# Vandermode/ELD

Measured on NVIDIA H100. Metric: raw frames/sec (noise+U-Net), higher is better.
Workload: dtype bf16

## Files before the change

eld_b200/csrc/conv3x3_thin.cuh:

```cuda
#pragma once
#include "conv_gemm.cuh"

namespace eld {

__host__ __device__ constexpr int thin_stg_bytes(int nt) { return 128 * nt * 2; }
constexpr int kThinMaxSlots = 4;
constexpr int kThinSmemBytes = 227 * 1024;

__device__ __forceinline__ uint32_t thin_stg_off(int m, int q) { return (uint32_t)(m * 64 + ((q ^ ((m >> 1) & 3)) << 4)); }

template <int NT, int KC>
__global__ void __launch_bounds__(kConvThreads, 1)
conv3x3_thin_kernel(const __grid_constant__ CUtensorMap tmA, const __grid_constant__ CUtensorMap tmOut,
                    const __grid_constant__ CUtensorMap tmOut2, const ConvGemmParams p)
{
    extern __shared__ uint8_t smem_raw[];
    const uint32_t raw = ptx::smem_u32(smem_raw);
    uint8_t* smem = smem_raw + (((raw + 1023u) & ~1023u) - raw);

    constexpr int row_bytes = KC * 2;
    constexpr int tap_bytes = NT * row_bytes;
    constexpr int slot_bytes = halo_slot_bytes(KC);
    constexpr int NC = NT / 32;
    uint8_t* b_s = smem;
    uint8_t* slots = smem + 9 * tap_bytes;
    uint64_t* full = reinterpret_cast<uint64_t*>(smem + p.bar_smem_off);
    uint64_t* empty = full + p.stages;
    uint64_t* b_full = empty + p.stages;
    float* s_bias = reinterpret_cast<float*>(smem + p.bias_smem_off);

    const int total_tiles = p.n_img * p.tiles_y * p.tiles_x;
    const int tiles_xy = p.tiles_x * p.tiles_y;

    if (threadIdx.x == 0) {
        ptx::prefetch_tmap(&tmA);
        ptx::prefetch_tmap(&tmOut);
        for (int s = 0; s < p.stages; ++s) { ptx::mbar_init(&full[s], 1); ptx::mbar_init(&empty[s], 4); }
        ptx::mbar_init(b_full, 1);
        ptx::fence_barrier_init();
    }
    if (p.bias)
        for (int i = threadIdx.x; i < p.n_total; i += kConvThreads) s_bias[i] = __ldg(p.bias + i);
    __syncthreads();
    ptx::grid_dep_wait();
    ptx::grid_dep_launch();

    if (threadIdx.x < 128) {
        if (threadIdx.x == 0) {
            ptx::mbar_arrive_expect_tx(b_full, (uint32_t)(9 * tap_bytes));
            for (int tap = 0; tap < 9; ++tap)
                ptx::bulk_load(b_s + tap * tap_bytes, p.b_ptr + (size_t)tap * p.b_rows * row_bytes, (uint32_t)tap_bytes, b_full);
            int s = 0;
            uint32_t ph = 0;
            for (int tile = blockIdx.x; tile < total_tiles; tile += gridDim.x) {
                const int img = tile / tiles_xy;
                const int rem = tile - img * tiles_xy;
                const int ty = rem / p.tiles_x, tx = rem - ty * p.tiles_x;
                const int x0 = tx * kConvTileW, y0 = ty * 8;
                ptx::mbar_wait(&empty[s], ph ^ 1u);
                uint8_t* sa = slots + (size_t)s * slot_bytes;
                ptx::mbar_arrive_expect_tx(&full[s], (uint32_t)slot_bytes);
                halo_load<KC>(sa, &tmA, &full[s], p.a_c0, x0, y0, img);
                if (++s == p.stages) { s = 0; ph ^= 1u; }
            }
        }
        return;
    }

    const int cg = __shfl_sync(0xffffffffu, (int)(threadIdx.x >> 7) - 1, 0);
    const int t = threadIdx.x & 127;
    const int lane = threadIdx.x & 31;
    const uint32_t layout = ptx::gmma_layout(row_bytes);
    const uint64_t desc0 = ptx::make_gmma_desc(0, 16, 8u * row_bytes, layout);
    const uint32_t b_base = ptx::smem_u32(b_s), slot_base = ptx::smem_u32(slots);
    uint8_t* stg = smem + p.stg_smem_off + cg * thin_stg_bytes(NT);
    const uint32_t stg_base = ptx::smem_u32(stg);
    const int wq = t >> 5, lr = lane >> 2, q = lane & 3;
    const size_t n_pix = (size_t)p.n_img * p.H * p.W;
    float bias[NT / 8][2];
#pragma unroll
    for (int j = 0; j < NT / 8; ++j) { bias[j][0] = p.bias ? s_bias[8 * j + 2 * q] : 0.f; bias[j][1] = p.bias ? s_bias[8 * j + 2 * q + 1] : 0.f; }
    ptx::mbar_wait(b_full, 0);
    for (int jt = cg;; jt += 2) {
        const int tile = blockIdx.x + jt * gridDim.x;
        if (tile >= total_tiles) break;
        const int s = jt % p.stages;
        const int img = tile / tiles_xy;
        const int rem = tile - img * tiles_xy;
        const int ty = rem / p.tiles_x, tx = rem - ty * p.tiles_x;
        const int x0 = tx * kConvTileW, y0 = ty * 8;
        long long pix[4];
#pragma unroll
        for (int u = 0; u < 4; ++u) {
            const int x = x0 + lr + 8 * (u & 1), y = y0 + 4 * (u >> 1) + wq;
            pix[u] = (x < p.W && y < p.H) ? ((long long)(img * p.H + y) * p.W + x) : -1;
        }
        ptx::mbar_wait(&full[s], (uint32_t)(jt / p.stages) & 1u);
        float acc[2][NT / 2];
        const uint32_t sa = slot_base + (uint32_t)(s * slot_bytes);
        ptx::wgmma_fence();
#pragma unroll
        for (int tap = 0; tap < 9; ++tap) {
            const uint32_t a_addr = sa + halo_tap_off(KC, tap);
            const uint64_t bd = ptx::desc_at(desc0, b_base + (uint32_t)(tap * tap_bytes));
#pragma unroll
            for (int k = 0; k < KC / 16; ++k) {
#pragma unroll
                for (int h = 0; h < 2; ++h) {
                    const uint64_t ad = ptx::desc_at(desc0, a_addr + (uint32_t)(h * 64 * row_bytes));
                    ptx::wgmma_bf16<NT, 0, 0>(acc[h], ad + 2u * k, bd + 2u * k, (tap | k) != 0 ? 1u : 0u);
                }
            }
        }
        ptx::wgmma_commit();
        uint32_t mneg[4][NC], mtie[4][NC];
        if (p.act == ACT_MASK && p.aux_slope) {
#pragma unroll
            for (int u = 0; u < 4; ++u)
#pragma unroll
                for (int c = 0; c < NC; ++c) {
                    const uint32_t* sw = p.aux_slope + (size_t)pix[u] * NC + c;
                    mneg[u][c] = pix[u] >= 0 ? __ldg(sw) : 0u;
                    mtie[u][c] = pix[u] >= 0 ? __ldg(sw + n_pix * NC) : 0u;
                }
        }
        ptx::wgmma_wait<0>();
        ptx::reg_fence(acc[0]);
        ptx::reg_fence(acc[1]);
        if (lane == 0) ptx::mbar_arrive(&empty[s]);

        if (p.act == ACT_MASK && !p.aux_slope) {
#pragma unroll
            for (int u = 0; u < 4; ++u)
#pragma unroll
                for (int c = 0; c < NC; ++c) {
                    mneg[u][c] = 0u; mtie[u][c] = 0u;
#pragma unroll
                    for (int jj = 0; jj < 4; ++jj) {
                        if (pix[u] < 0) continue;
                        const int k = 4 * jj + q;
                        const uint32_t w = __ldg(reinterpret_cast<const uint32_t*>(
                            p.aux + (size_t)pix[u] * p.aux_pitch + (p.aux_c0 + 32 * c + 2 * k)));
                        uint32_t n, tc;
                        ptx::slope_classes(w, n, tc);
                        mneg[u][c] |= (n >> (15 - k)) & (0x00010001u << k);
                        mtie[u][c] |= (tc >> (15 - k)) & (0x00010001u << k);
                    }
                }
        }

        uint32_t wv[2][NT / 8][2];
#pragma unroll
        for (int h = 0; h < 2; ++h)
#pragma unroll
            for (int j = 0; j < NT / 8; ++j)
#pragma unroll
                for (int i = 0; i < 2; ++i) {
                    float v[2] = { acc[h][4 * j + 2 * i], acc[h][4 * j + 2 * i + 1] };
#pragma unroll
                    for (int c = 0; c < 2; ++c) {
                        if (p.bias) v[c] += bias[j][c];
                        if (p.act == ACT_LRELU) {
                            v[c] = fmaxf(v[c], 0.2f * v[c]);
                        } else if (p.act == ACT_MASK) {
                            const int u = 2 * h + i, b = 4 * (j & 3) + q + 16 * c;
                            v[c] *= lrelu_slope(mneg[u][j >> 2], mtie[u][j >> 2], b, kMaskNeg);
                        }
                    }
                    const __nv_bfloat162 b2 = __floats2bfloat162_rn(v[0], v[1]);
                    wv[h][j][i] = *reinterpret_cast<const uint32_t*>(&b2);
                }
        if (p.slope_out) {
            uint32_t sn[4][NC], st[4][NC];
#pragma unroll
            for (int u = 0; u < 4; ++u)
#pragma unroll
                for (int c = 0; c < NC; ++c) {
                    sn[u][c] = 0u; st[u][c] = 0u;
#pragma unroll
                    for (int jj = 0; jj < 4; ++jj) {
                        const int k = 4 * jj + q;
                        uint32_t n, tc;
                        ptx::slope_classes(wv[u >> 1][4 * c + jj][u & 1], n, tc);
                        sn[u][c] |= (n >> (15 - k)) & (0x00010001u << k);
                        st[u][c] |= (tc >> (15 - k)) & (0x00010001u << k);
                    }
#pragma unroll
                    for (int o = 1; o <= 2; o <<= 1) {
                        sn[u][c] |= __shfl_xor_sync(0xffffffffu, sn[u][c], o);
                        st[u][c] |= __shfl_xor_sync(0xffffffffu, st[u][c], o);
                    }
                }
#pragma unroll
            for (int u = 0; u < 4; ++u)
                if (u == q && pix[u] >= 0) {
                    uint32_t* sw = p.slope_out + (size_t)pix[u] * NC;
#pragma unroll
                    for (int c = 0; c < NC; ++c) { sw[c] = sn[u][c]; sw[n_pix * NC + c] = st[u][c]; }
                }
        }

        if (t == 0) ptx::bulk_wait_read<0>();
        ptx::bar_sync(1 + cg, 128);
#pragma unroll
        for (int h = 0; h < 2; ++h)
#pragma unroll
            for (int c = 0; c < NC; ++c)
#pragma unroll
                for (int jp = 0; jp < 2; ++jp) {
                    const int g = lane >> 3;
                    const int m = 64 * h + 16 * wq + 8 * (g & 1) + (lane & 7);
                    const int j0 = 4 * c + 2 * jp;
                    ptx::stmatrix_x4(stg_base + (uint32_t)(c * 128 * 64) + thin_stg_off(m, 2 * jp + (g >> 1)),
                                     wv[h][j0][0], wv[h][j0][1], wv[h][j0 + 1][0], wv[h][j0 + 1][1]);
                }
        ptx::fence_proxy_async();
        ptx::bar_sync(1 + cg, 128);
        if (t == 0) {
#pragma unroll
            for (int c = 0; c < NC; ++c) {
                const bool second = p.out_split && 32 * c >= p.out_split;
                ptx::tma_store_5d(second ? &tmOut2 : &tmOut, stg + c * 128 * 64,
                                  second ? 32 * c - p.out_split : p.out_c0 + 32 * c, x0, y0, img, 0);
            }
            ptx::bulk_commit();
        }
        if (p.pool_out) {
#pragma unroll
            for (int it = t; it < 128 * NC; it += 128) {
                const int qq = it & 3, px = (it >> 2) & 7, py = (it >> 5) & 3, c = it >> 7;
                const uint8_t* blk = stg + c * 128 * 64;
                uint32_t w[4][4];
#pragma unroll
                for (int d = 0; d < 4; ++d) {
                    const uint4 v = *reinterpret_cast<const uint4*>(blk + thin_stg_off(16 * (2 * py + (d >> 1)) + 2 * px + (d & 1), qq));
                    w[d][0] = v.x; w[d][1] = v.y; w[d][2] = v.z; w[d][3] = v.w;
                }
                uint32_t pw[4];
#pragma unroll
                for (int jj = 0; jj < 4; ++jj) pw[jj] = bf2_max(bf2_max(w[0][jj], w[1][jj]), bf2_max(w[2][jj], w[3][jj]));
                const int x = x0 + 2 * px, y = y0 + 2 * py;
                const bool in_img = x < p.W && y < p.H;
                const size_t ppix = (size_t)(img * (p.H >> 1) + (y >> 1)) * (p.W >> 1) + (x >> 1);
                if (in_img)
                    *reinterpret_cast<uint4*>(p.pool_out + ppix * p.pool_pitch + 32 * c + 8 * qq) = make_uint4(pw[0], pw[1], pw[2], pw[3]);
                if (p.pool_code) {
                    uint32_t code[12];
#pragma unroll
                    for (int d = 0; d < 4; ++d) {
                        code[d] = 0u; code[4 + d] = 0u; code[8 + d] = 0u;
#pragma unroll
                        for (int jj = 0; jj < 4; ++jj) {
                            const int k = 4 * qq + jj;
                            const uint32_t ne = __hne2_mask(*reinterpret_cast<const __nv_bfloat162*>(&w[d][jj]),
                                                            *reinterpret_cast<const __nv_bfloat162*>(&pw[jj]));
                            uint32_t n, tc;
                            ptx::slope_classes(w[d][jj], n, tc);
                            code[d] |= (ne >> (15 - k)) & (0x00010001u << k);
                            code[4 + d] |= (n >> (15 - k)) & (0x00010001u << k);
                            code[8 + d] |= (tc >> (15 - k)) & (0x00010001u << k);
                        }
                    }
#pragma unroll
                    for (int e = 0; e < 12; ++e) {
                        code[e] |= __shfl_xor_sync(0xffffffffu, code[e], 1);
                        code[e] |= __shfl_xor_sync(0xffffffffu, code[e], 2);
                    }
                    const size_t rec = ppix * (size_t)(p.pool_pitch >> 5) + (size_t)c;
                    const size_t recs = (size_t)p.n_img * (p.H >> 1) * (p.W >> 1) * (size_t)(p.pool_pitch >> 5);
                    uint32_t* dst = qq == 2 ? p.pool_code + recs * 8 + rec * 4 : p.pool_code + rec * 8 + 4 * qq;
#pragma unroll
                    for (int g = 0; g < 3; ++g)
                        if (in_img && qq == g)
                            *reinterpret_cast<uint4*>(dst) = make_uint4(code[4 * g], code[4 * g + 1], code[4 * g + 2], code[4 * g + 3]);
                }
            }
        }
    }
    if (t == 0) ptx::bulk_wait<0>();
}

}
```

eld_b200/csrc/unet_prims.cu:

```cuda
#include "common.cuh"
#include <algorithm>
#include <cstdlib>
#include <cstdio>
#include "conv_gemm.cuh"
#include "conv3x3_thin.cuh"
#include "conv3x3_wide.cuh"
#include "wgrad_gemm.cuh"
#include "wgrad_thin.cuh"
#include "first_conv.cuh"
#include "unet_prims.h"

namespace eld {

using ConvKernel = void (*)(CUtensorMap, ConvGemmParams);
using WgradKernel = void (*)(CUtensorMap, CUtensorMap, WgradParams);
using WgradThinKernel = void (*)(CUtensorMap, CUtensorMap, WgradThinParams);
using FirstConvKernel = void (*)(CUtensorMap, CUtensorMap, FirstConvParams);
static const ConvKernel kConvGemm[3] = { conv_gemm_kernel<32>, conv_gemm_kernel<64>, conv_gemm_kernel<128> };
using ConvThinKernel = void (*)(CUtensorMap, CUtensorMap, CUtensorMap, ConvGemmParams);
static const ConvThinKernel kConvThin[2][2] = { { conv3x3_thin_kernel<32, 32>, conv3x3_thin_kernel<32, 64> },
                                                { conv3x3_thin_kernel<64, 32>, conv3x3_thin_kernel<64, 64> } };
static const ConvKernel kConvWide[3][2] = { { conv3x3_wide_kernel<32, 32>, conv3x3_wide_kernel<32, 64> },
                                            { conv3x3_wide_kernel<64, 32>, conv3x3_wide_kernel<64, 64> },
                                            { conv3x3_wide_kernel<128, 32>, conv3x3_wide_kernel<128, 64> } };
static const WgradKernel kWgradGemm[3] = { wgrad_gemm_kernel<32>, wgrad_gemm_kernel<64>, wgrad_gemm_kernel<128> };
static const WgradThinKernel kWgradThin[2][2] = { { conv3x3_wgrad_thin_kernel<32, 32>, conv3x3_wgrad_thin_kernel<32, 64> },
                                                  { conv3x3_wgrad_thin_kernel<64, 32>, conv3x3_wgrad_thin_kernel<64, 64> } };
static const FirstConvKernel kFirstConv[2] = { first_conv_kernel<false>, first_conv_kernel<true> };

static int encode(eld_ctx* ctx, CUtensorMap* map, const void* ptr, int rank, const cuuint64_t* dims,
                  const cuuint64_t* strides_bytes, const cuuint32_t* box, int inner_bytes,
                  CUtensorMapDataType dtype = CU_TENSOR_MAP_DATA_TYPE_BFLOAT16)
{
    cuuint32_t estr[5] = { 1, 1, 1, 1, 1 };
    CUtensorMapSwizzle sw = inner_bytes == 128 ? CU_TENSOR_MAP_SWIZZLE_128B
                          : inner_bytes == 64  ? CU_TENSOR_MAP_SWIZZLE_64B
                          : inner_bytes == 32  ? CU_TENSOR_MAP_SWIZZLE_32B : CU_TENSOR_MAP_SWIZZLE_NONE;
    CUresult r = ctx->encode_tiled(map, dtype, (cuuint32_t)rank, const_cast<void*>(ptr),
                                   dims, strides_bytes, box, estr, CU_TENSOR_MAP_INTERLEAVE_NONE, sw,
                                   CU_TENSOR_MAP_L2_PROMOTION_L2_256B, CU_TENSOR_MAP_FLOAT_OOB_FILL_NONE);
    if (r != CUDA_SUCCESS) {
        set_error("cuTensorMapEncodeTiled failed (%d): rank %d dims %llu,%llu,%llu box %u,%u,%u inner %d B",
                  (int)r, rank, (unsigned long long)dims[0], (unsigned long long)dims[1],
                  (unsigned long long)(rank > 2 ? dims[2] : 0), box[0], box[1], rank > 2 ? box[2] : 0, inner_bytes);
        return ELD_E_CUDA;
    }
    return ELD_OK;
}

static int encode_nhwc(eld_ctx* ctx, CUtensorMap* map, const void* t, int pitch, int n, int H, int W,
                       int box_c, int box_w, int box_h)
{
    const cuuint64_t eb = 2;
    cuuint64_t dims[5] = { (cuuint64_t)pitch, (cuuint64_t)W, (cuuint64_t)H, (cuuint64_t)n, 1 };
    cuuint64_t str[4] = { pitch * eb, (cuuint64_t)W * pitch * eb, (cuuint64_t)H * W * pitch * eb,
                          (cuuint64_t)n * H * W * pitch * eb };
    cuuint32_t box[5] = { (cuuint32_t)box_c, (cuuint32_t)box_w, (cuuint32_t)box_h, 1, 1 };
    return encode(ctx, map, t, 5, dims, str, box, box_c * 2);
}

static int encode_subpixel(eld_ctx* ctx, CUtensorMap* map, const void* t, int pitch, int n, int H, int W,
                           int box_c, int box_rows)
{
    const cuuint64_t eb = 2;
    cuuint64_t dims[5] = { (cuuint64_t)pitch, 2, (cuuint64_t)W, 2, (cuuint64_t)n * H };
    cuuint64_t str[4] = { pitch * eb, 2 * pitch * eb, (cuuint64_t)2 * W * pitch * eb, (cuuint64_t)4 * W * pitch * eb };
    cuuint32_t box[5] = { (cuuint32_t)box_c, 1, 16, 1, (cuuint32_t)box_rows };
    return encode(ctx, map, t, 5, dims, str, box, box_c * 2);
}

template <typename Kernel, typename... Args>
static int launch(eld_ctx* ctx, Kernel kernel, int grid, int block, size_t smem, cudaStream_t st, Args... args)
{
    ELD_CHECK_CUDA(launch_pdl(kernel, grid, block, smem, st, args...));
    ELD_CHECK_CUDA(cudaGetLastError());
    count_launch(ctx);
    return ELD_OK;
}

static int conv_gemm_params(const GemmOp& op, ConvGemmParams& p)
{
    const int n_total = op.kind == GEMM_DECONV ? 4 * op.cout : op.cout;
    const bool store = op.kind != GEMM_DECONV;
    ELD_REQUIRE(op.cin % 32 == 0, "conv tile: cin=%d must be a multiple of 32", op.cin);
    ELD_REQUIRE(n_total % 32 == 0, "conv tile: GEMM N=%d must be a multiple of 32", n_total);
    ELD_REQUIRE(op.a_pitch % 8 == 0, "conv tile: the input pitch must be a multiple of 8 channels");
    ELD_REQUIRE(op.out_pitch % 16 == 0 && op.out_c0 % 16 == 0 && (reinterpret_cast<uintptr_t>(op.out) & 31) == 0,
                "conv tile: output pitch / first channel must be multiples of 16 channels and the tensor 32-byte aligned");
    ELD_REQUIRE(op.aux == nullptr || (op.aux_pitch % 16 == 0 && op.aux_c0 % 16 == 0 && (reinterpret_cast<uintptr_t>(op.aux) & 31) == 0),
                "conv tile: mask-source pitch / first channel must be multiples of 16 channels and the tensor 32-byte aligned");
    ELD_REQUIRE(op.pool_out == nullptr || (op.pool_pitch % 16 == 0 && (reinterpret_cast<uintptr_t>(op.pool_out) & 31) == 0),
                "conv tile: pooled-output pitch must be a multiple of 16 channels and the tensor 32-byte aligned");
    p.n_img = op.n_img; p.H = op.H; p.W = op.W;
    p.tiles_x = (op.W + 15) / 16; p.tiles_y = (op.H + 7) / 8;
    p.taps = op.kind == GEMM_CONV3X3 ? 9 : op.kind == GEMM_DECONV ? 1 : 4;
    p.a_mode = op.kind == GEMM_DECONV_DGRAD ? A_GATHER : A_CONV;
    p.cin = op.cin; p.a_c0 = op.a_c0;
    p.kc = (op.cin % 64 == 0) ? 64 : 32;
    p.n_total = n_total;
    p.epi_mode = store ? EPI_STORE : EPI_SHUFFLE; p.act = op.act;
    p.out = static_cast<__nv_bfloat16*>(op.out); p.out_pitch = op.out_pitch; p.out_c0 = op.out_c0;
    p.bias = op.bias;
    p.aux = static_cast<const __nv_bfloat16*>(op.aux); p.aux_pitch = op.aux_pitch; p.aux_c0 = op.aux_c0;
    ELD_REQUIRE(op.aux_slope == nullptr || (op.act == ACT_MASK && store), "conv tile: slope words are a mask source of a plain store epilogue");
    ELD_REQUIRE(op.slope_out == nullptr || (op.act == ACT_LRELU && store && op.out_split == 0),
                "conv tile: slope words are written behind LeakyReLU by a plain store epilogue");
    p.aux_slope = static_cast<const uint32_t*>(op.aux_slope); p.slope_out = static_cast<uint32_t*>(op.slope_out);
    p.cout = op.cout;
    ELD_REQUIRE(op.pool_out == nullptr || (store && op.H % 2 == 0 && op.W % 2 == 0),
                "conv tile: the fused max pool needs a plain store epilogue and even H, W");
    p.pool_out = static_cast<__nv_bfloat16*>(op.pool_out); p.pool_pitch = op.pool_pitch;
    ELD_REQUIRE(op.pool_code == nullptr || (op.pool_out && op.pool_pitch % 32 == 0 && (reinterpret_cast<uintptr_t>(op.pool_code) & 31) == 0),
                "conv tile: the pool code needs the fused pool, a multiple of 32 channels and a 32-byte aligned buffer");
    p.pool_code = static_cast<uint32_t*>(op.pool_code);
    ELD_REQUIRE(op.out_split == 0 || (store && op.out2 && op.out_split % 32 == 0 && op.out2_pitch % 16 == 0 &&
                                     (reinterpret_cast<uintptr_t>(op.out2) & 31) == 0),
                "conv tile: split store needs a plain store epilogue, a second tensor and a split at a multiple of 32 columns");
    p.out2 = static_cast<__nv_bfloat16*>(op.out2); p.out2_pitch = op.out2_pitch; p.out_split = op.out_split;
    ELD_REQUIRE(op.b_block_rows == 0 || (op.b_block_rows % 32 == 0 && op.b_block_rows <= 256 &&
                                         (n_total <= op.b_block_rows || op.b_block_rows == 256) && op.aux_slope == nullptr),
                "conv tile: a row prefix of the packed operand needs whole 32-row groups of its blocks and no slope-word mask");
    ELD_REQUIRE(op.b_block_rows != 0 || n_total <= 256 || n_total % 256 == 0,
                "conv tile: GEMM N=%d above 256 must be a multiple of 256", n_total);
    p.b_rows = op.b_block_rows ? op.b_block_rows : (n_total <= 256 ? n_total : 256);
    p.n_tile = (n_total % 128 == 0) ? 128 : (n_total % 64 == 0) ? 64 : 32;
    const int n_bias = store ? n_total : op.cout;
    ELD_REQUIRE(n_bias <= 1024, "conv tile: %d bias entries exceed the 4 KB shared-memory copy", n_bias);
    p.cout_shift = 0;
    if (!store) {
        ELD_REQUIRE(op.cout >= 32 && (op.cout & (op.cout - 1)) == 0, "deconv tile: cout=%d must be a power of two >= 32", op.cout);
        while ((1 << p.cout_shift) < op.cout) ++p.cout_shift;
    }
    p.b_ptr = static_cast<const uint8_t*>(op.b);
    return ELD_OK;
}

static int launch_conv3x3(eld_ctx* ctx, const GemmOp& op, ConvGemmParams& p, cudaStream_t st)
{
    CUtensorMap tmA;
    { int rc = encode_nhwc(ctx, &tmA, op.a, op.a_pitch, op.n_img, op.H, op.W, p.kc, kConvTileW, kHaloRows); if (rc) return rc; }
    const int rb = p.kc * 2;
    const int slot_bytes = halo_slot_bytes(p.kc);
    if ((op.cin == 32 || op.cin == 64) && (p.n_total == 32 || p.n_total == 64)) {
        const int stg = thin_stg_bytes(p.n_tile);
        const int fixed = 9 * p.n_tile * rb + 2 * stg + 256;
        int slots = (kThinSmemBytes - 1024 - fixed - 256) / slot_bytes;
        if (slots > kThinMaxSlots) slots = kThinMaxSlots;
        ELD_REQUIRE(slots >= 2, "thin conv tile: no room for two halo slots");
        p.stages = slots;
        p.stg_smem_off = 9 * p.n_tile * rb + slots * slot_bytes;
        p.bias_smem_off = p.stg_smem_off + 2 * stg;
        p.bar_smem_off = p.bias_smem_off + 256;
        const size_t smem = 1024 + (size_t)p.bar_smem_off + 256;
        CUtensorMap tmOut, tmOut2;
        { int rc = encode_nhwc(ctx, &tmOut, op.out, op.out_pitch, op.n_img, op.H, op.W, 32, kConvTileW, 8); if (rc) return rc; }
        tmOut2 = tmOut;
        if (op.out_split) { int rc = encode_nhwc(ctx, &tmOut2, op.out2, op.out2_pitch, op.n_img, op.H, op.W, 32, kConvTileW, 8); if (rc) return rc; }
        const int total_tiles = op.n_img * p.tiles_x * p.tiles_y;
        return launch(ctx, kConvThin[p.n_tile / 64][p.kc / 64], std::min(total_tiles, ctx->num_sms), kConvThreads, smem, st,
                      tmA, tmOut, tmOut2, p);
    }
    const int stg_bytes = 2 * 64 * kConvStg * 4;
    const int b_bytes = p.n_tile * rb;
    const int fixed = kWideHaloSlots * slot_bytes + stg_bytes + 4096;
    int wstages = (kThinSmemBytes - 1024 - 256 - fixed) / b_bytes;
    if (wstages > 8) wstages = 8;
    ELD_REQUIRE(wstages >= 2, "wide conv tile: no room for two weight stages");
    p.stages = wstages;
    p.stg_smem_off = kWideHaloSlots * slot_bytes + wstages * b_bytes;
    p.bias_smem_off = p.stg_smem_off + stg_bytes;
    p.bar_smem_off = p.bias_smem_off + 4096;
    const size_t smem = 1024 + (size_t)p.bar_smem_off + 256;
    const int total_tiles = op.n_img * p.tiles_x * p.tiles_y * (p.n_total / p.n_tile);
    return launch(ctx, kConvWide[p.n_tile / 64][p.kc / 64], std::min(total_tiles, ctx->num_sms), kConvThreads, smem, st,
                  tmA, p);
}

static int launch_deconv(eld_ctx* ctx, const GemmOp& op, ConvGemmParams& p, cudaStream_t st)
{
    ELD_REQUIRE(op.kind == GEMM_DECONV || (op.H % 8 == 0 && op.W % 16 == 0),
                "deconv dgrad tile: H=%d must be a multiple of 8 and W=%d of 16", op.H, op.W);
    CUtensorMap tmA;
    { int rc = op.kind == GEMM_DECONV ? encode_nhwc(ctx, &tmA, op.a, op.a_pitch, op.n_img, op.H, op.W, p.kc, 16, 8)
                                      : encode_subpixel(ctx, &tmA, op.a, op.a_pitch, op.n_img, op.H, op.W, p.kc, 8);
      if (rc) return rc; }
    const int rb = p.kc * 2;
    const int stg_bytes = 2 * 64 * kConvStg * 4;
    const int stage_bytes = 128 * rb + p.n_tile * rb;
    int stages = (200 * 1024 - stg_bytes - 4096) / stage_bytes;
    if (stages > 8) stages = 8;
    if (stages < 2) stages = 2;
    p.stages = stages;
    p.stg_smem_off = stages * stage_bytes;
    p.bias_smem_off = p.stg_smem_off + stg_bytes;
    p.bar_smem_off = p.bias_smem_off + 4096;
    const int total_tiles = op.n_img * p.tiles_x * p.tiles_y * (p.n_total / p.n_tile);
    const size_t smem = 1024  + (size_t)p.bar_smem_off + 256 ;
    return launch(ctx, kConvGemm[p.n_tile / 64], std::min(total_tiles, ctx->num_sms), kConvThreads, smem, st, tmA, p);
}

int launch_conv_gemm(eld_ctx* ctx, const GemmOp& op, cudaStream_t st)
{
    ConvGemmParams p{};
    { int rc = conv_gemm_params(op, p); if (rc) return rc; }
    return op.kind == GEMM_CONV3X3 ? launch_conv3x3(ctx, op, p, st) : launch_deconv(ctx, op, p, st);
}

static int encode_frame(eld_ctx* ctx, CUtensorMap* map, const float* x, int cin, int n, int H, int W)
{
    ELD_REQUIRE((reinterpret_cast<uintptr_t>(x) & 15) == 0, "first conv tile: the input frame must be 16-byte aligned");
    cuuint64_t dims[5] = { (cuuint64_t)W * 2, (cuuint64_t)H, (cuuint64_t)cin, (cuuint64_t)n, 1 };
    cuuint64_t str[4] = { (cuuint64_t)W * 4, (cuuint64_t)H * W * 4, (cuuint64_t)cin * H * W * 4, (cuuint64_t)n * cin * H * W * 4 };
    cuuint32_t box[5] = { 64, 10, 4, 1, 1 };
    return encode(ctx, map, x, 5, dims, str, box, 128);
}

static size_t first_conv_smem(bool wgrad)
{
    const size_t slot = kFcRaw + (wgrad ? kFcQTile : 0);
    const size_t stg = wgrad ? 0 : ((128 * kFcStg * 4 + 1023) & ~1023);
    return 1024 + 4096 + 2 * (kFcATile + kFcRing * slot + stg) + 512;
}

int launch_first_conv(eld_ctx* ctx, const float* x, int cin, const void* w_img, const float* bias, void* out, int out_pitch,
                      int n, int H, int W, cudaStream_t st, void* slope_out)
{
    ELD_REQUIRE(H % 8 == 0 && W % 16 == 0, "first conv tile: H=%d must be a multiple of 8 and W=%d of 16", H, W);
    FirstConvParams p{};
    p.x = x; p.n_img = n; p.H = H; p.W = W; p.tiles_x = W / 16; p.tiles_y = H / 8; p.cin = cin;
    p.w_img = static_cast<const uint8_t*>(w_img); p.bias = bias;
    p.out = static_cast<__nv_bfloat16*>(out); p.out_pitch = out_pitch; p.slope_out = static_cast<uint32_t*>(slope_out);
    const int total = n * p.tiles_x * p.tiles_y;
    CUtensorMap tmX;
    { int rc = encode_frame(ctx, &tmX, x, cin, n, H, W); if (rc) return rc; }
    return launch(ctx, kFirstConv[0], std::min(total, ctx->num_sms), kFcThreads, first_conv_smem(false), st, tmX, tmX, p);
}

int launch_first_conv_wgrad(eld_ctx* ctx, const float* x, int cin, const void* dz, int dz_pitch, float* dw, float* db,
                            int n, int H, int W, cudaStream_t st)
{
    ELD_REQUIRE(H % 8 == 0 && W % 16 == 0, "first conv wgrad tile: H=%d must be a multiple of 8 and W=%d of 16", H, W);
    FirstConvParams p{};
    p.x = x; p.n_img = n; p.H = H; p.W = W; p.tiles_x = W / 16; p.tiles_y = H / 8; p.cin = cin;
    p.dw = dw; p.db = db;
    CUtensorMap tmQ;
    { int rc = encode_nhwc(ctx, &tmQ, dz, dz_pitch, n, H, W, 32, 16, 8); if (rc) return rc; }
    const int total = n * p.tiles_x * p.tiles_y;
    CUtensorMap tmX;
    { int rc = encode_frame(ctx, &tmX, x, cin, n, H, W); if (rc) return rc; }
    return launch(ctx, kFirstConv[1], std::min(total, ctx->num_sms), kFcThreads, first_conv_smem(true), st, tmX, tmQ, p);
}

static size_t first_conv_dgrad_smem() { return 1024 + kDgStages * halo_slot_bytes(32) + kDgB + 2 * kDgStages * 8; }

int launch_first_conv_dgrad(eld_ctx* ctx, const void* dz, const float* w, int cin, float* dx, int n, int H, int W,
                            cudaStream_t st)
{
    ELD_REQUIRE(H % 8 == 0 && W % 16 == 0, "first conv dgrad tile: H=%d must be a multiple of 8 and W=%d of 16", H, W);
    ELD_REQUIRE(cin >= 1 && cin <= 8, "first conv dgrad tile: cin=%d must be 1..8 (wgmma N = 8)", cin);
    FirstConvParams p{};
    p.n_img = n; p.H = H; p.W = W; p.tiles_x = W / 16; p.tiles_y = H / 8; p.cin = cin;
    p.w = w; p.dx = dx;
    CUtensorMap tmZ;
    { int rc = encode_nhwc(ctx, &tmZ, dz, 32, n, H, W, 32, kConvTileW, kHaloRows); if (rc) return rc; }
    const int total = n * p.tiles_x * p.tiles_y;
    return launch(ctx, first_conv_dgrad_kernel, std::min(total, ctx->num_sms), kDgThreads, first_conv_dgrad_smem(), st, tmZ, p);
}

int init_gemm_kernels(eld_ctx* ctx)
{
    const auto attr = cudaFuncAttributeMaxDynamicSharedMemorySize;
    ELD_CHECK_CUDA(cudaSetDevice(ctx->device));
    ELD_CHECK_CUDA(cudaFuncSetAttribute(first_conv_dgrad_kernel, attr, (int)first_conv_dgrad_smem()));
    for (int wgrad = 0; wgrad < 2; ++wgrad)
        ELD_CHECK_CUDA(cudaFuncSetAttribute(kFirstConv[wgrad], attr, (int)first_conv_smem(wgrad)));
    for (auto k : kConvGemm) ELD_CHECK_CUDA(cudaFuncSetAttribute(k, attr, 220 * 1024));
    for (auto& nt : kConvThin) for (auto k : nt) ELD_CHECK_CUDA(cudaFuncSetAttribute(k, attr, kThinSmemBytes));
    for (auto& nt : kConvWide) for (auto k : nt) ELD_CHECK_CUDA(cudaFuncSetAttribute(k, attr, kThinSmemBytes));
    for (auto k : kWgradGemm) ELD_CHECK_CUDA(cudaFuncSetAttribute(k, attr, 220 * 1024));
    for (auto& nt : kWgradThin) for (auto k : nt) ELD_CHECK_CUDA(cudaFuncSetAttribute(k, attr, kThinSmemBytes));
    return ELD_OK;
}

static int launch_wgrad_thin(eld_ctx* ctx, const WgradOp& op, cudaStream_t st)
{
    ELD_REQUIRE(op.out_tco == 0 || (reinterpret_cast<uintptr_t>(op.dw) & 15) == 0,
                "thin wgrad tile: the [tap][ci][co] gradient must be 16-byte aligned");
    ELD_REQUIRE(op.db == nullptr || (reinterpret_cast<uintptr_t>(op.db) & 15) == 0,
                "thin wgrad tile: the bias gradient must be 16-byte aligned");
    WgradThinParams p{};
    p.n_img = op.n_img; p.H = op.H; p.W = op.W;
    p.tiles_x = op.W / 16; p.tiles_y = (op.H + 7) / 8;
    p.p_c0 = op.p_c0; p.q_c0 = op.q_c0; p.cin = op.p_ch; p.cout = op.q_ch;
    const int kc = std::min(op.p_ch, 64), nt = std::min(op.q_ch, 64);
    p.ci_blocks = op.p_ch / kc; p.co_blocks = op.q_ch / nt;
    p.dw = op.dw; p.out_tco = op.out_tco; p.db = op.db;
    const int slot_bytes = wgrad_thin_slot_bytes(kc, nt);
    int stages = (kThinSmemBytes - 1024 - 256) / slot_bytes;
    if (stages > kThinMaxSlots) stages = kThinMaxSlots;
    ELD_REQUIRE(stages >= 2, "thin wgrad tile: no room for two stages");
    p.stages = stages;

    CUtensorMap tmP, tmQ;
    { int rc = encode_nhwc(ctx, &tmP, op.p, op.p_pitch, op.n_img, op.H, op.W, kc, kConvTileW, kHaloRows); if (rc) return rc; }
    { int rc = encode_nhwc(ctx, &tmQ, op.q, op.q_pitch, op.n_img, op.H, op.W, nt, 16, 8); if (rc) return rc; }
    const size_t smem = 1024 + (size_t)stages * slot_bytes + 256;
    const int total_tiles = op.n_img * p.tiles_x * p.tiles_y;
    const int blocks = p.ci_blocks * p.co_blocks;
    p.splits = std::min(std::max(1, ctx->num_sms / blocks), total_tiles);
    return launch(ctx, kWgradThin[nt / 64][kc / 64], blocks * p.splits, kWgThinThreads, smem, st, tmP, tmQ, p);
}

int launch_wgrad(eld_ctx* ctx, const WgradOp& op, cudaStream_t st)
// ... 277 lines not shown
```

eld_b200/csrc/wgmma.cuh:

```cuda
#pragma once
#include <cstdint>
#include <cuda_runtime.h>
#include <cuda.h>

namespace eld {
namespace ptx {

__device__ __forceinline__ uint32_t smem_u32(const void* p) { return (uint32_t)__cvta_generic_to_shared(p); }

__device__ __forceinline__ void mbar_init(uint64_t* bar, uint32_t count)
{
    asm volatile("mbarrier.init.shared::cta.b64 [%0], %1;" ::"r"(smem_u32(bar)), "r"(count));
}
__device__ __forceinline__ void fence_barrier_init()
{
    asm volatile("fence.mbarrier_init.release.cluster;" ::: "memory");
}
__device__ __forceinline__ void fence_proxy_async()
{
    asm volatile("fence.proxy.async.shared::cta;" ::: "memory");
}
__device__ __forceinline__ void mbar_arrive_expect_tx(uint64_t* bar, uint32_t bytes)
{
    asm volatile("mbarrier.arrive.expect_tx.shared::cta.b64 _, [%0], %1;" ::"r"(smem_u32(bar)), "r"(bytes) : "memory");
}
__device__ __forceinline__ void mbar_arrive(uint64_t* bar)
{
    asm volatile("mbarrier.arrive.shared::cta.b64 _, [%0];" ::"r"(smem_u32(bar)) : "memory");
}
__device__ __forceinline__ bool mbar_try_wait(uint64_t* bar, uint32_t parity)
{
    uint32_t ok;
    asm volatile(
        "{\n\t.reg .pred p;\n\t"
        "mbarrier.try_wait.parity.shared::cta.b64 p, [%1], %2;\n\t"
        "selp.u32 %0, 1, 0, p;\n\t}"
        : "=r"(ok) : "r"(smem_u32(bar)), "r"(parity) : "memory");
    return ok != 0;
}
__device__ __forceinline__ void mbar_wait(uint64_t* bar, uint32_t parity)
{
    while (!mbar_try_wait(bar, parity)) { }
}

__device__ __forceinline__ void bar_sync(uint32_t id, uint32_t count)
{
    asm volatile("bar.sync %0, %1;" ::"r"(id), "r"(count) : "memory");
}

__device__ __forceinline__ void grid_dep_wait() { asm volatile("griddepcontrol.wait;" ::: "memory"); }
__device__ __forceinline__ void grid_dep_launch() { asm volatile("griddepcontrol.launch_dependents;" ::: "memory"); }

__device__ __forceinline__ void prefetch_tmap(const CUtensorMap* m)
{
    asm volatile("prefetch.tensormap [%0];" ::"l"(m) : "memory");
}
__device__ __forceinline__ void tma_load_5d(void* dst, const CUtensorMap* m, uint64_t* bar,
                                            int c0, int c1, int c2, int c3, int c4)
{
    asm volatile(
        "cp.async.bulk.tensor.5d.shared::cluster.global.mbarrier::complete_tx::bytes [%0], [%1, {%3, %4, %5, %6, %7}], [%2];"
        ::"r"(smem_u32(dst)), "l"(m), "r"(smem_u32(bar)), "r"(c0), "r"(c1), "r"(c2), "r"(c3), "r"(c4) : "memory");
}

__device__ __forceinline__ void bulk_load(void* dst, const void* src, uint32_t bytes, uint64_t* bar)
{
    asm volatile("cp.async.bulk.shared::cluster.global.mbarrier::complete_tx::bytes [%0], [%1], %2, [%3];"
                 ::"r"(smem_u32(dst)), "l"(src), "r"(bytes), "r"(smem_u32(bar)) : "memory");
}

__device__ __forceinline__ void tma_store_5d(const CUtensorMap* m, const void* src, int c0, int c1, int c2, int c3, int c4)
{
    asm volatile("cp.async.bulk.tensor.5d.global.shared::cta.bulk_group [%0, {%2, %3, %4, %5, %6}], [%1];"
                 ::"l"(m), "r"(smem_u32(src)), "r"(c0), "r"(c1), "r"(c2), "r"(c3), "r"(c4) : "memory");
}
__device__ __forceinline__ void bulk_commit() { asm volatile("cp.async.bulk.commit_group;" ::: "memory"); }
template <int N>
__device__ __forceinline__ void bulk_wait_read() { asm volatile("cp.async.bulk.wait_group.read %0;" ::"n"(N) : "memory"); }
template <int N>
__device__ __forceinline__ void bulk_wait() { asm volatile("cp.async.bulk.wait_group %0;" ::"n"(N) : "memory"); }

__device__ __forceinline__ void stmatrix_x4(uint32_t addr, uint32_t r0, uint32_t r1, uint32_t r2, uint32_t r3)
{
    asm volatile("stmatrix.sync.aligned.m8n8.x4.shared.b16 [%0], {%1, %2, %3, %4};"
                 ::"r"(addr), "r"(r0), "r"(r1), "r"(r2), "r"(r3) : "memory");
}

__device__ __forceinline__ void st_global_32B(void* p, const uint32_t w[8])
{
    asm volatile("st.global.v4.b32 [%0], {%1,%2,%3,%4};\n\tst.global.v4.b32 [%0+16], {%5,%6,%7,%8};"
                 :: "l"(p), "r"(w[0]), "r"(w[1]), "r"(w[2]), "r"(w[3]), "r"(w[4]), "r"(w[5]), "r"(w[6]), "r"(w[7]) : "memory");
}
__device__ __forceinline__ void ld_global_nc_32B(const void* p, uint32_t w[8])
{
    asm volatile("ld.global.nc.v4.b32 {%0,%1,%2,%3}, [%8];\n\tld.global.nc.v4.b32 {%4,%5,%6,%7}, [%8+16];"
                 : "=r"(w[0]), "=r"(w[1]), "=r"(w[2]), "=r"(w[3]), "=r"(w[4]), "=r"(w[5]), "=r"(w[6]), "=r"(w[7]) : "l"(p));
}

__device__ __forceinline__ uint64_t desc_at(uint64_t desc, uint32_t smem_addr)
{
    return desc | (uint64_t)((smem_addr & 0x3FFFFu) >> 4);
}
__device__ __forceinline__ uint64_t make_gmma_desc(uint32_t smem_addr, uint32_t lbo_bytes, uint32_t sbo_bytes, uint32_t layout)
{
    uint64_t d = desc_at(0, smem_addr);
    d |= (uint64_t)((lbo_bytes >> 4) & 0x3FFFu) << 16;
    d |= (uint64_t)((sbo_bytes >> 4) & 0x3FFFu) << 32;
    d |= (uint64_t)(layout & 3u) << 62;
    return d;
}
constexpr uint32_t GMMA_SW128 = 1, GMMA_SW64 = 2;
__host__ __device__ constexpr uint32_t gmma_layout(int row_bytes) { return row_bytes == 128 ? GMMA_SW128 : GMMA_SW64; }

__device__ __forceinline__ void wgmma_fence() { asm volatile("wgmma.fence.sync.aligned;" ::: "memory"); }
__device__ __forceinline__ void wgmma_commit() { asm volatile("wgmma.commit_group.sync.aligned;" ::: "memory"); }
template <int N>
__device__ __forceinline__ void wgmma_wait() { asm volatile("wgmma.wait_group.sync.aligned %0;" ::"n"(N) : "memory"); }
template <int R>
__device__ __forceinline__ void reg_fence(float (&d)[R])
{
#pragma unroll
    for (int i = 0; i < R; ++i) asm volatile("" : "+f"(d[i])::"memory");
}

template <int TA, int TB>
__device__ __forceinline__ void wgmma_m64n8k16(float (&d)[4], uint64_t a_desc, uint64_t b_desc, uint32_t scale_d)
{
    asm volatile(
        "{\n\t.reg .pred p;\n\tsetp.ne.b32 p, %6, 0;\n\t"
        "wgmma.mma_async.sync.aligned.m64n8k16.f32.bf16.bf16 {%0,%1,%2,%3}, %4, %5, p, 1, 1, %7, %8;\n\t}"
        : "+f"(d[0]), "+f"(d[1]), "+f"(d[2]), "+f"(d[3])
        : "l"(a_desc), "l"(b_desc), "r"(scale_d), "n"(TA), "n"(TB) : "memory");
}
template <int TA, int TB>
__device__ __forceinline__ void wgmma_m64n32k16(float (&d)[16], uint64_t a_desc, uint64_t b_desc, uint32_t scale_d)
{
    asm volatile(
        "{\n\t.reg .pred p;\n\tsetp.ne.b32 p, %18, 0;\n\t"
        "wgmma.mma_async.sync.aligned.m64n32k16.f32.bf16.bf16 {%0,%1,%2,%3,%4,%5,%6,%7,%8,%9,%10,%11,%12,%13,%14,%15}, %16, %17, p, 1, 1, %19, %20;\n\t}"
        : "+f"(d[0]), "+f"(d[1]), "+f"(d[2]), "+f"(d[3]), "+f"(d[4]), "+f"(d[5]), "+f"(d[6]), "+f"(d[7]), "+f"(d[8]), "+f"(d[9]), "+f"(d[10]), "+f"(d[11]), "+f"(d[12]), "+f"(d[13]), "+f"(d[14]), "+f"(d[15])
        : "l"(a_desc), "l"(b_desc), "r"(scale_d), "n"(TA), "n"(TB) : "memory");
}
template <int TA, int TB>
__device__ __forceinline__ void wgmma_m64n64k16(float (&d)[32], uint64_t a_desc, uint64_t b_desc, uint32_t scale_d)
{
    asm volatile(
        "{\n\t.reg .pred p;\n\tsetp.ne.b32 p, %34, 0;\n\t"
        "wgmma.mma_async.sync.aligned.m64n64k16.f32.bf16.bf16 {%0,%1,%2,%3,%4,%5,%6,%7,%8,%9,%10,%11,%12,%13,%14,%15,%16,%17,%18,%19,%20,%21,%22,%23,%24,%25,%26,%27,%28,%29,%30,%31}, %32, %33, p, 1, 1, %35, %36;\n\t}"
        : "+f"(d[0]), "+f"(d[1]), "+f"(d[2]), "+f"(d[3]), "+f"(d[4]), "+f"(d[5]), "+f"(d[6]), "+f"(d[7]), "+f"(d[8]), "+f"(d[9]), "+f"(d[10]), "+f"(d[11]), "+f"(d[12]), "+f"(d[13]), "+f"(d[14]), "+f"(d[15]), "+f"(d[16]), "+f"(d[17]), "+f"(d[18]), "+f"(d[19]), "+f"(d[20]), "+f"(d[21]), "+f"(d[22]), "+f"(d[23]), "+f"(d[24]), "+f"(d[25]), "+f"(d[26]), "+f"(d[27]), "+f"(d[28]), "+f"(d[29]), "+f"(d[30]), "+f"(d[31])
        : "l"(a_desc), "l"(b_desc), "r"(scale_d), "n"(TA), "n"(TB) : "memory");
}
template <int TA, int TB>
__device__ __forceinline__ void wgmma_m64n128k16(float (&d)[64], uint64_t a_desc, uint64_t b_desc, uint32_t scale_d)
{
    asm volatile(
        "{\n\t.reg .pred p;\n\tsetp.ne.b32 p, %66, 0;\n\t"
        "wgmma.mma_async.sync.aligned.m64n128k16.f32.bf16.bf16 {%0,%1,%2,%3,%4,%5,%6,%7,%8,%9,%10,%11,%12,%13,%14,%15,%16,%17,%18,%19,%20,%21,%22,%23,%24,%25,%26,%27,%28,%29,%30,%31,%32,%33,%34,%35,%36,%37,%38,%39,%40,%41,%42,%43,%44,%45,%46,%47,%48,%49,%50,%51,%52,%53,%54,%55,%56,%57,%58,%59,%60,%61,%62,%63}, %64, %65, p, 1, 1, %67, %68;\n\t}"
        : "+f"(d[0]), "+f"(d[1]), "+f"(d[2]), "+f"(d[3]), "+f"(d[4]), "+f"(d[5]), "+f"(d[6]), "+f"(d[7]), "+f"(d[8]), "+f"(d[9]), "+f"(d[10]), "+f"(d[11]), "+f"(d[12]), "+f"(d[13]), "+f"(d[14]), "+f"(d[15]), "+f"(d[16]), "+f"(d[17]), "+f"(d[18]), "+f"(d[19]), "+f"(d[20]), "+f"(d[21]), "+f"(d[22]), "+f"(d[23]), "+f"(d[24]), "+f"(d[25]), "+f"(d[26]), "+f"(d[27]), "+f"(d[28]), "+f"(d[29]), "+f"(d[30]), "+f"(d[31]), "+f"(d[32]), "+f"(d[33]), "+f"(d[34]), "+f"(d[35]), "+f"(d[36]), "+f"(d[37]), "+f"(d[38]), "+f"(d[39]), "+f"(d[40]), "+f"(d[41]), "+f"(d[42]), "+f"(d[43]), "+f"(d[44]), "+f"(d[45]), "+f"(d[46]), "+f"(d[47]), "+f"(d[48]), "+f"(d[49]), "+f"(d[50]), "+f"(d[51]), "+f"(d[52]), "+f"(d[53]), "+f"(d[54]), "+f"(d[55]), "+f"(d[56]), "+f"(d[57]), "+f"(d[58]), "+f"(d[59]), "+f"(d[60]), "+f"(d[61]), "+f"(d[62]), "+f"(d[63])
        : "l"(a_desc), "l"(b_desc), "r"(scale_d), "n"(TA), "n"(TB) : "memory");
}

template <int N, int TA, int TB>
__device__ __forceinline__ void wgmma_bf16(float (&d)[N / 2], uint64_t a_desc, uint64_t b_desc, uint32_t scale_d)
{
    if constexpr (N == 32) wgmma_m64n32k16<TA, TB>(d, a_desc, b_desc, scale_d);
    else if constexpr (N == 64) wgmma_m64n64k16<TA, TB>(d, a_desc, b_desc, scale_d);
    else wgmma_m64n128k16<TA, TB>(d, a_desc, b_desc, scale_d);
}

__device__ __forceinline__ uint32_t gather_msb16(const uint32_t (&w)[16])
{
    uint32_t a[4] = { 0u, 0u, 0u, 0u };
#pragma unroll
    for (int j = 0; j < 16; ++j) a[j & 3] |= (w[j] >> (15 - j)) & (0x00010001u << j);
    return (a[0] | a[1]) | (a[2] | a[3]);
}

__device__ __forceinline__ void slope_classes(uint32_t w, uint32_t& n, uint32_t& t)
{
    const uint32_t mag = w & 0x7FFF7FFFu;
    t = (mag + 0x00800080u) | (0x80008000u - mag);
    n = (mag + 0x007F007Fu) | (w & ~t);
}
__device__ __forceinline__ void slope_words(const uint32_t (&w)[16], uint32_t& neg, uint32_t& tie)
{
    uint32_t n[16], t[16];
#pragma unroll
    for (int j = 0; j < 16; ++j) slope_classes(w[j], n[j], t[j]);
    neg = gather_msb16(n);
    tie = gather_msb16(t);
}

}

__device__ __forceinline__ float lrelu_slope(uint32_t neg, uint32_t tie, int b, float neg_slope)
{
    const bool n = (neg >> b) & 1u, t = (tie >> b) & 1u;
    return t ? (n ? 1.2f : 0.6f) : (n ? neg_slope : 1.0f);
}
constexpr float kMaskNeg = 0.6f - 0.4f;
}
```

Before: 1105.

## Use three consumer warpgroups in thin conv, TMA-load slope masks, rebalance registers

The thin 3x3 conv kernel goes from two to three consumer warpgroups, each with its own per-stage full barrier. The producer drops its registers via setmaxnreg so the consumers can take more. Slope mask words are now brought into shared memory by a 3D TMA load on the same barrier as the halo, replacing per-thread global loads. The output staging buffer is processed in smaller chunks so three staging buffers fit in shared memory. This should hide more latency, at the cost of fewer halo slots and a new requirement that H and W be whole tiles when slope masks are used.

```diff
diff --git a/eld_b200/csrc/conv3x3_thin.cuh b/eld_b200/csrc/conv3x3_thin.cuh
--- a/eld_b200/csrc/conv3x3_thin.cuh
+++ b/eld_b200/csrc/conv3x3_thin.cuh
@@ -3,16 +3,22 @@
 
 namespace eld {
 
-__host__ __device__ constexpr int thin_stg_bytes(int nt) { return 128 * nt * 2; }
+constexpr int kThinConsumers = 3;
+constexpr int kThinThreads = 128 * (1 + kThinConsumers);
+__host__ __device__ constexpr int thin_stg_blocks(int nt, int kc) { return nt == 64 && kc == 64 ? 1 : nt / 32; }
+__host__ __device__ constexpr int thin_stg_bytes(int nt, int kc) { return thin_stg_blocks(nt, kc) * 128 * 32 * 2; }
+__host__ __device__ constexpr int thin_slope_bytes(int nt) { return 2 * 8 * 16 * (nt / 32) * 4; }
 constexpr int kThinMaxSlots = 4;
 constexpr int kThinSmemBytes = 227 * 1024;
+constexpr int kThinProducerRegs = 24;
 
 __device__ __forceinline__ uint32_t thin_stg_off(int m, int q) { return (uint32_t)(m * 64 + ((q ^ ((m >> 1) & 3)) << 4)); }
 
 template <int NT, int KC>
-__global__ void __launch_bounds__(kConvThreads, 1)
+__global__ void __launch_bounds__(kThinThreads, 1)
 conv3x3_thin_kernel(const __grid_constant__ CUtensorMap tmA, const __grid_constant__ CUtensorMap tmOut,
-                    const __grid_constant__ CUtensorMap tmOut2, const ConvGemmParams p)
+                    const __grid_constant__ CUtensorMap tmOut2, const __grid_constant__ CUtensorMap tmSlope,
+                    const ConvGemmParams p)
 {
     extern __shared__ uint8_t smem_raw[];
     const uint32_t raw = ptx::smem_u32(smem_raw);
@@ -22,10 +28,15 @@
     constexpr int tap_bytes = NT * row_bytes;
     constexpr int slot_bytes = halo_slot_bytes(KC);
     constexpr int NC = NT / 32;
+    constexpr int CG = kThinConsumers;
+    constexpr int SB = thin_stg_blocks(NT, KC);
+    constexpr int slope_bytes = thin_slope_bytes(NT);
+    const bool slope_box = p.act == ACT_MASK && p.aux_slope;
     uint8_t* b_s = smem;
     uint8_t* slots = smem + 9 * tap_bytes;
+    uint8_t* slope_s = slots + p.stages * slot_bytes;
     uint64_t* full = reinterpret_cast<uint64_t*>(smem + p.bar_smem_off);
-    uint64_t* empty = full + p.stages;
+    uint64_t* empty = full + p.stages * CG;
     uint64_t* b_full = empty + p.stages;
     float* s_bias = reinterpret_cast<float*>(smem + p.bias_smem_off);
 
@@ -35,22 +46,27 @@
     if (threadIdx.x == 0) {
         ptx::prefetch_tmap(&tmA);
         ptx::prefetch_tmap(&tmOut);
-        for (int s = 0; s < p.stages; ++s) { ptx::mbar_init(&full[s], 1); ptx::mbar_init(&empty[s], 4); }
+        if (slope_box) ptx::prefetch_tmap(&tmSlope);
+        for (int s = 0; s < p.stages; ++s) {
+            for (int c = 0; c < CG; ++c) ptx::mbar_init(&full[s * CG + c], 1);
+            ptx::mbar_init(&empty[s], 4);
+        }
         ptx::mbar_init(b_full, 1);
         ptx::fence_barrier_init();
     }
     if (p.bias)
-        for (int i = threadIdx.x; i < p.n_total; i += kConvThreads) s_bias[i] = __ldg(p.bias + i);
+        for (int i = threadIdx.x; i < p.n_total; i += kThinThreads) s_bias[i] = __ldg(p.bias + i);
     __syncthreads();
     ptx::grid_dep_wait();
     ptx::grid_dep_launch();
 
     if (threadIdx.x < 128) {
+        asm volatile("setmaxnreg.dec.sync.aligned.u32 %0;" ::"n"(kThinProducerRegs));
         if (threadIdx.x == 0) {
             ptx::mbar_arrive_expect_tx(b_full, (uint32_t)(9 * tap_bytes));
             for (int tap = 0; tap < 9; ++tap)
                 ptx::bulk_load(b_s + tap * tap_bytes, p.b_ptr + (size_t)tap * p.b_rows * row_bytes, (uint32_t)tap_bytes, b_full);
-            int s = 0;
+            int s = 0, c = 0;
             uint32_t ph = 0;
             for (int tile = blockIdx.x; tile < total_tiles; tile += gridDim.x) {
                 const int img = tile / tiles_xy;
@@ -59,21 +75,25 @@
                 const int x0 = tx * kConvTileW, y0 = ty * 8;
                 ptx::mbar_wait(&empty[s], ph ^ 1u);
                 uint8_t* sa = slots + (size_t)s * slot_bytes;
-                ptx::mbar_arrive_expect_tx(&full[s], (uint32_t)slot_bytes);
-                halo_load<KC>(sa, &tmA, &full[s], p.a_c0, x0, y0, img);
+                uint64_t* bar = &full[s * CG + c];
+                ptx::mbar_arrive_expect_tx(bar, (uint32_t)(slot_bytes + (slope_box ? slope_bytes : 0)));
+                halo_load<KC>(sa, &tmA, bar, p.a_c0, x0, y0, img);
+                if (slope_box) ptx::tma_load_3d(slope_s + s * slope_bytes, &tmSlope, bar, x0 * NC, img * p.H + y0, 0);
                 if (++s == p.stages) { s = 0; ph ^= 1u; }
+                if (++c == CG) c = 0;
             }
         }
         return;
     }
 
+    asm volatile("setmaxnreg.inc.sync.aligned.u32 %0;" ::"n"(NT == 32 ? 152 : 160));
     const int cg = __shfl_sync(0xffffffffu, (int)(threadIdx.x >> 7) - 1, 0);
     const int t = threadIdx.x & 127;
     const int lane = threadIdx.x & 31;
     const uint32_t layout = ptx::gmma_layout(row_bytes);
     const uint64_t desc0 = ptx::make_gmma_desc(0, 16, 8u * row_bytes, layout);
     const uint32_t b_base = ptx::smem_u32(b_s), slot_base = ptx::smem_u32(slots);
-    uint8_t* stg = smem + p.stg_smem_off + cg * thin_stg_bytes(NT);
+    uint8_t* stg = smem + p.stg_smem_off + cg * thin_stg_bytes(NT, KC);
     const uint32_t stg_base = ptx::smem_u32(stg);
     const int wq = t >> 5, lr = lane >> 2, q = lane & 3;
     const size_t n_pix = (size_t)p.n_img * p.H * p.W;
@@ -81,7 +101,8 @@
 #pragma unroll
     for (int j = 0; j < NT / 8; ++j) { bias[j][0] = p.bias ? s_bias[8 * j + 2 * q] : 0.f; bias[j][1] = p.bias ? s_bias[8 * j + 2 * q + 1] : 0.f; }
     ptx::mbar_wait(b_full, 0);
-    for (int jt = cg;; jt += 2) {
+    uint32_t full_ph = 0;
+    for (int jt = cg;; jt += CG) {
         const int tile = blockIdx.x + jt * gridDim.x;
         if (tile >= total_tiles) break;
         const int s = jt % p.stages;
@@ -95,7 +116,8 @@
             const int x = x0 + lr + 8 * (u & 1), y = y0 + 4 * (u >> 1) + wq;
             pix[u] = (x < p.W && y < p.H) ? ((long long)(img * p.H + y) * p.W + x) : -1;
         }
-        ptx::mbar_wait(&full[s], (uint32_t)(jt / p.stages) & 1u);
+        ptx::mbar_wait(&full[s * CG + cg], (full_ph >> s) & 1u);
+        full_ph ^= 1u << s;
         float acc[2][NT / 2];
         const uint32_t sa = slot_base + (uint32_t)(s * slot_bytes);
         ptx::wgmma_fence();
@@ -114,19 +136,21 @@
         }
         ptx::wgmma_commit();
         uint32_t mneg[4][NC], mtie[4][NC];
-        if (p.act == ACT_MASK && p.aux_slope) {
+        if (slope_box) {
+            const uint32_t* sw = reinterpret_cast<const uint32_t*>(slope_s + s * slope_bytes);
 #pragma unroll
             for (int u = 0; u < 4; ++u)
 #pragma unroll
                 for (int c = 0; c < NC; ++c) {
-                    const uint32_t* sw = p.aux_slope + (size_t)pix[u] * NC + c;
-                    mneg[u][c] = pix[u] >= 0 ? __ldg(sw) : 0u;
-                    mtie[u][c] = pix[u] >= 0 ? __ldg(sw + n_pix * NC) : 0u;
+                    const int w = ((4 * (u >> 1) + wq) * kConvTileW + lr + 8 * (u & 1)) * NC + c;
+                    mneg[u][c] = sw[w];
+                    mtie[u][c] = sw[128 * NC + w];
                 }
         }
         ptx::wgmma_wait<0>();
         ptx::reg_fence(acc[0]);
         ptx::reg_fence(acc[1]);
+        if (slope_box) __syncwarp();
         if (lane == 0) ptx::mbar_arrive(&empty[s]);
 
         if (p.act == ACT_MASK && !p.aux_slope) {
@@ -200,36 +224,38 @@
                 }
         }
 
+#pragma unroll
+        for (int c0 = 0; c0 < NC; c0 += SB) {
         if (t == 0) ptx::bulk_wait_read<0>();
         ptx::bar_sync(1 + cg, 128);
 #pragma unroll
         for (int h = 0; h < 2; ++h)
 #pragma unroll
-            for (int c = 0; c < NC; ++c)
+            for (int c = c0; c < c0 + SB; ++c)
 #pragma unroll
                 for (int jp = 0; jp < 2; ++jp) {
                     const int g = lane >> 3;
                     const int m = 64 * h + 16 * wq + 8 * (g & 1) + (lane & 7);
                     const int j0 = 4 * c + 2 * jp;
-                    ptx::stmatrix_x4(stg_base + (uint32_t)(c * 128 * 64) + thin_stg_off(m, 2 * jp + (g >> 1)),
+                    ptx::stmatrix_x4(stg_base + (uint32_t)((c - c0) * 128 * 64) + thin_stg_off(m, 2 * jp + (g >> 1)),
                                      wv[h][j0][0], wv[h][j0][1], wv[h][j0 + 1][0], wv[h][j0 + 1][1]);
                 }
         ptx::fence_proxy_async();
         ptx::bar_sync(1 + cg, 128);
         if (t == 0) {
 #pragma unroll
-            for (int c = 0; c < NC; ++c) {
+            for (int c = c0; c < c0 + SB; ++c) {
                 const bool second = p.out_split && 32 * c >= p.out_split;
-                ptx::tma_store_5d(second ? &tmOut2 : &tmOut, stg + c * 128 * 64,
+                ptx::tma_store_5d(second ? &tmOut2 : &tmOut, stg + (c - c0) * 128 * 64,
                                   second ? 32 * c - p.out_split : p.out_c0 + 32 * c, x0, y0, img, 0);
             }
             ptx::bulk_commit();
         }
         if (p.pool_out) {
 #pragma unroll
-            for (int it = t; it < 128 * NC; it += 128) {
-                const int qq = it & 3, px = (it >> 2) & 7, py = (it >> 5) & 3, c = it >> 7;
-                const uint8_t* blk = stg + c * 128 * 64;
+            for (int it = t; it < 128 * SB; it += 128) {
+                const int qq = it & 3, px = (it >> 2) & 7, py = (it >> 5) & 3, c = c0 + (it >> 7);
+                const uint8_t* blk = stg + (it >> 7) * 128 * 64;
                 uint32_t w[4][4];
 #pragma unroll
                 for (int d = 0; d < 4; ++d) {
@@ -276,6 +302,7 @@
                 }
             }
         }
+        }
     }
     if (t == 0) ptx::bulk_wait<0>();
 }
diff --git a/eld_b200/csrc/unet_prims.cu b/eld_b200/csrc/unet_prims.cu
--- a/eld_b200/csrc/unet_prims.cu
+++ b/eld_b200/csrc/unet_prims.cu
@@ -17,7 +17,7 @@
 using WgradThinKernel = void (*)(CUtensorMap, CUtensorMap, WgradThinParams);
 using FirstConvKernel = void (*)(CUtensorMap, CUtensorMap, FirstConvParams);
 static const ConvKernel kConvGemm[3] = { conv_gemm_kernel<32>, conv_gemm_kernel<64>, conv_gemm_kernel<128> };
-using ConvThinKernel = void (*)(CUtensorMap, CUtensorMap, CUtensorMap, ConvGemmParams);
+using ConvThinKernel = void (*)(CUtensorMap, CUtensorMap, CUtensorMap, CUtensorMap, ConvGemmParams);
 static const ConvThinKernel kConvThin[2][2] = { { conv3x3_thin_kernel<32, 32>, conv3x3_thin_kernel<32, 64> },
                                                 { conv3x3_thin_kernel<64, 32>, conv3x3_thin_kernel<64, 64> } };
 static const ConvKernel kConvWide[3][2] = { { conv3x3_wide_kernel<32, 32>, conv3x3_wide_kernel<32, 64> },
@@ -142,23 +142,36 @@
     const int rb = p.kc * 2;
     const int slot_bytes = halo_slot_bytes(p.kc);
     if ((op.cin == 32 || op.cin == 64) && (p.n_total == 32 || p.n_total == 64)) {
-        const int stg = thin_stg_bytes(p.n_tile);
-        const int fixed = 9 * p.n_tile * rb + 2 * stg + 256;
-        int slots = (kThinSmemBytes - 1024 - fixed - 256) / slot_bytes;
+        const int cg = kThinConsumers, slope_bytes = thin_slope_bytes(p.n_tile);
+        const int stg = thin_stg_bytes(p.n_tile, p.kc);
+        const int fixed = 9 * p.n_tile * rb + cg * stg + 256;
+        int slots = (kThinSmemBytes - 1024 - fixed - 256) / (slot_bytes + slope_bytes);
         if (slots > kThinMaxSlots) slots = kThinMaxSlots;
         ELD_REQUIRE(slots >= 2, "thin conv tile: no room for two halo slots");
         p.stages = slots;
-        p.stg_smem_off = 9 * p.n_tile * rb + slots * slot_bytes;
-        p.bias_smem_off = p.stg_smem_off + 2 * stg;
+        p.stg_smem_off = 9 * p.n_tile * rb + slots * (slot_bytes + slope_bytes);
+        p.bias_smem_off = p.stg_smem_off + cg * stg;
         p.bar_smem_off = p.bias_smem_off + 256;
         const size_t smem = 1024 + (size_t)p.bar_smem_off + 256;
         CUtensorMap tmOut, tmOut2;
         { int rc = encode_nhwc(ctx, &tmOut, op.out, op.out_pitch, op.n_img, op.H, op.W, 32, kConvTileW, 8); if (rc) return rc; }
         tmOut2 = tmOut;
         if (op.out_split) { int rc = encode_nhwc(ctx, &tmOut2, op.out2, op.out2_pitch, op.n_img, op.H, op.W, 32, kConvTileW, 8); if (rc) return rc; }
+        CUtensorMap tmSlope = tmA;
+        if (p.aux_slope) {
+            const int nc = p.n_tile / 32;
+            ELD_REQUIRE(op.H % 8 == 0 && op.W % kConvTileW == 0 && (reinterpret_cast<uintptr_t>(op.aux_slope) & 15) == 0,
+                        "thin conv tile: a slope-word mask needs whole 8 x 16 tiles (H=%d, W=%d) and 16-byte aligned words",
+                        op.H, op.W);
+            const cuuint64_t dims[3] = { (cuuint64_t)op.W * nc, (cuuint64_t)op.n_img * op.H, 2 };
+            const cuuint64_t str[2] = { (cuuint64_t)op.W * nc * 4, (cuuint64_t)op.n_img * op.H * op.W * nc * 4 };
+            const cuuint32_t box[3] = { (cuuint32_t)(kConvTileW * nc), 8, 2 };
+            int rc = encode(ctx, &tmSlope, op.aux_slope, 3, dims, str, box, 0 , CU_TENSOR_MAP_DATA_TYPE_UINT32);
+            if (rc) return rc;
+        }
         const int total_tiles = op.n_img * p.tiles_x * p.tiles_y;
-        return launch(ctx, kConvThin[p.n_tile / 64][p.kc / 64], std::min(total_tiles, ctx->num_sms), kConvThreads, smem, st,
-                      tmA, tmOut, tmOut2, p);
+        return launch(ctx, kConvThin[p.n_tile / 64][p.kc / 64], std::min(total_tiles, ctx->num_sms),
+                      kThinThreads, smem, st, tmA, tmOut, tmOut2, tmSlope, p);
     }
     const int stg_bytes = 2 * 64 * kConvStg * 4;
     const int b_bytes = p.n_tile * rb;
diff --git a/eld_b200/csrc/wgmma.cuh b/eld_b200/csrc/wgmma.cuh
--- a/eld_b200/csrc/wgmma.cuh
+++ b/eld_b200/csrc/wgmma.cuh
@@ -61,6 +61,13 @@
     asm volatile(
         "cp.async.bulk.tensor.5d.shared::cluster.global.mbarrier::complete_tx::bytes [%0], [%1, {%3, %4, %5, %6, %7}], [%2];"
         ::"r"(smem_u32(dst)), "l"(m), "r"(smem_u32(bar)), "r"(c0), "r"(c1), "r"(c2), "r"(c3), "r"(c4) : "memory");
+}
+
+__device__ __forceinline__ void tma_load_3d(void* dst, const CUtensorMap* m, uint64_t* bar, int c0, int c1, int c2)
+{
+    asm volatile(
+        "cp.async.bulk.tensor.3d.shared::cluster.global.mbarrier::complete_tx::bytes [%0], [%1, {%3, %4, %5}], [%2];"
+        ::"r"(smem_u32(dst)), "l"(m), "r"(smem_u32(bar)), "r"(c0), "r"(c1), "r"(c2) : "memory");
 }
 
 __device__ __forceinline__ void bulk_load(void* dst, const void* src, uint32_t bytes, uint64_t* bar)
```

After: 1141 (median of 6 runs). 1.03x the previous value.
